# humeniuka/semiclassical

Hardware: AMD Instinct MI355X
Metric: trajectory-steps/sec + wall-time to converged C(t), anharmonic-AS D=60 (higher is better)
Workload: dtype f64

## Files before the change

### include/semiclassical_hip.h

```cpp
#ifndef SEMICLASSICAL_HIP_H
#define SEMICLASSICAL_HIP_H

#include <stdint.h>

#ifdef __cplusplus
extern "C" {
#endif

#define SC_ABI_VERSION        18

#define SC_OK                 0
#define SC_ERR_BAD_ARGUMENT  -1
#define SC_ERR_UNSUPPORTED   -2
#define SC_ERR_LAUNCH        -3

#define SC_POT_MORSE          1
#define SC_POT_HARMONIC_SEP   2
#define SC_POT_EPS_MORSE      3
#define SC_POT_HARMONIC_DENSE 4

typedef struct sc_potential {
    int32_t kind;
    int32_t dim;
    const double *par0;
// ... 71 lines not shown
    double *ksum;
    double *ssum;
} sc_dense_scratch;

int         sc_version(void);
const char *sc_last_error(void);
int sc_abi_version(void);
int sc_struct_size(const char *name);
int sc_tuning_build(void);

int sc_step_grid(int64_t n, int32_t dim);
int sc_correlate_grid(int64_t n, int32_t dim);

int sc_mono_convert(const sc_state *st, int32_t to_layout, void *stream);

int sc_state_from_reference(const double *y, const sc_state *st, void *stream);
int sc_state_to_reference(const sc_state *st, double *y, void *stream);

int sc_sample_initial(const sc_state *st, const double *ilz, const double *z0, int32_t dprime, double prob0,
                      uint64_t seed, uint64_t subsequence, int64_t first, int32_t init_state, double *zi_t,
                      double *probi, double *xi_out, void *stream);

int sc_hk_step(const sc_potential *pot, const sc_state *st, const sc_hk_consts *hk,
               double dt, int32_t mode, double *energy_partials, void *stream);

typedef struct sc_multi_scratch {
    double *work, *qp_mid, *act_mid, *c2_mid, *sgn_mid;
    int32_t *unrepaired;
} sc_multi_scratch;
int sc_hk_step_multi_supported(const sc_potential *pot, const sc_state *st, const sc_hk_consts *hk);
int sc_hk_step_multi(const sc_potential *pot, const sc_state *st, const sc_hk_consts *hk, const sc_multi_scratch *ms,
                     double dt, double *energy_partials, void *stream);

int sc_overlap(const sc_overlap_consts *oc, const double *qp, int64_t n, double *out, void *stream);

int sc_nac_initial(const sc_nac_consts *nc, const double *zi, int64_t n, double *nacq, void *stream);

int sc_hk_correlate(const sc_state *st, const sc_overlap_consts *ovl_t0, const sc_nac_consts *nc,
                    const double *vi, const double *probi, const double *nacq, double mc_norm,
                    double *cq_out, double *kq_out, double *partials, void *stream);

int sc_hk_correlate_m(const sc_state *st, const sc_overlap_consts *ovl_t0, const sc_nac_consts *nc,
                      const double *vi, const double *probi, const double *nacq, double mc_norm,
                      double *cq_out, double *kq_out, double *partials, double *moment_partials, void *stream);
int sc_term_moments_grid(int64_t n);
int sc_term_moments(const double *cq, const double *kq, int64_t n, double *moment_partials, void *stream);
int sc_reduce_moments(const double *moment_partials, int32_t n_rows, double *moments, void *stream);
int sc_reduce_slot_moments_at(const double *corr_partials, int32_t n_corr, const double *moment_partials, int32_t n_mom,
                              double *slots, double *moments, int64_t *cursor, void *stream);

int sc_reduce_slot(const double *corr_partials, int32_t n_corr, const double *energy_partials, int32_t n_energy_blocks,
                   double n_energy, double *slot, void *stream);

int sc_reduce_slot_at(const double *corr_partials, int32_t n_corr, double *slots, int64_t *cursor, void *stream);

int sc_hk_run_slots(int64_t n, int32_t dim);
int sc_hk_run_supported(const sc_potential *pot, const sc_hk_consts *hk, const sc_overlap_consts *ovl_t0);
int sc_hk_run(const sc_potential *pot, const sc_state *st, const sc_hk_consts *hk, const sc_overlap_consts *ovl_t0,
              const sc_nac_consts *nc, const double *vi, const double *probi, const double *nacq, double mc_norm,
              double dt, int32_t nsteps, double *partials, double *slots_out, double *elog, void *stream);

int64_t sc_hk_run_scratch_doubles(int64_t n, int32_t dim, int32_t nsteps, int32_t moments);
int sc_hk_run_m(const sc_potential *pot, const sc_state *st, const sc_hk_consts *hk, const sc_overlap_consts *ovl_t0,
                const sc_nac_consts *nc, const double *vi, const double *probi, const double *nacq, double mc_norm,
                double dt, int32_t nsteps, double *partials, double *slots_out, double *elog, double *moments_out, void *stream);

// ... 92 lines not shown
```

### semiclassical_amd/_lib.py

```python
import ctypes as C
import os

HERE = os.path.dirname(os.path.abspath(__file__))
LIB_PATH = os.environ.get("SC_LIB_PATH") or os.path.join(HERE, "libsemiclassical_hip.so")

c_double_p = C.c_void_p


class sc_potential(C.Structure):
    _fields_ = [("kind", C.c_int32), ("dim", C.c_int32),
                ("par0", c_double_p), ("par1", c_double_p), ("par2", c_double_p),
                ("scalar0", C.c_double), ("inv_mass", c_double_p),
                ("lin_prop", c_double_p), ("lin_dt", C.c_double)]


class sc_state(C.Structure):
    _fields_ = [("n", C.c_int64), ("dim", C.c_int32), ("mono_layout", C.c_int32),
                ("qp", c_double_p), ("act", c_double_p), ("mono", c_double_p),
                ("c2", c_double_p), ("sgn", c_double_p), ("work", c_double_p), ("flags", C.c_void_p)]


class sc_hk_consts(C.Structure):
    _fields_ = [("dim", C.c_int32), ("dprime", C.c_int32), ("diag", C.c_int32), ("real_lr", C.c_int32),
                ("st", c_double_p), ("si", c_double_p),
# ... 39 lines not shown


class sc_dense_scratch(C.Structure):
    _fields_ = [("hess", c_double_p), ("kprev", c_double_p), ("ksum", c_double_p), ("ssum", c_double_p)]


SC_POT_MORSE, SC_POT_HARMONIC_SEP, SC_POT_EPS_MORSE, SC_POT_HARMONIC_DENSE = 1, 2, 3, 4
SEPARABLE_KINDS = (SC_POT_MORSE, SC_POT_HARMONIC_SEP, SC_POT_EPS_MORSE)
SC_MONO_ROWMAJOR, SC_MONO_TILED16 = 0, 1

P = C.POINTER
ABI_VERSION = 18
STRUCTS = (sc_potential, sc_state, sc_hk_consts, sc_overlap_consts, sc_nac_consts, sc_wm_consts, sc_gdml_model,
           sc_dense_scratch, sc_multi_scratch)

SIGNATURES = {
    "sc_version": (C.c_int, []),
    "sc_abi_version": (C.c_int, []),
    "sc_struct_size": (C.c_int, [C.c_char_p]),
    "sc_tuning_build": (C.c_int, []),
    "sc_last_error": (C.c_char_p, []),
    "sc_step_grid": (C.c_int, [C.c_int64, C.c_int32]),
    "sc_correlate_grid": (C.c_int, [C.c_int64, C.c_int32]),
    "sc_mono_convert": (C.c_int, [P(sc_state), C.c_int32, C.c_void_p]),
    "sc_state_from_reference": (C.c_int, [c_double_p, P(sc_state), C.c_void_p]),
    "sc_state_to_reference": (C.c_int, [P(sc_state), c_double_p, C.c_void_p]),
    "sc_sample_initial": (C.c_int, [P(sc_state), c_double_p, c_double_p, C.c_int32, C.c_double, C.c_uint64, C.c_uint64,
                                    C.c_int64, C.c_int32, c_double_p, c_double_p, c_double_p, C.c_void_p]),
    "sc_hk_step": (C.c_int, [P(sc_potential), P(sc_state), P(sc_hk_consts), C.c_double, C.c_int32,
                             c_double_p, C.c_void_p]),
    "sc_hk_step_multi_supported": (C.c_int, [P(sc_potential), P(sc_state), P(sc_hk_consts)]),
    "sc_hk_step_multi": (C.c_int, [P(sc_potential), P(sc_state), P(sc_hk_consts), P(sc_multi_scratch), C.c_double, c_double_p,
                                   C.c_void_p]),
    "sc_overlap": (C.c_int, [P(sc_overlap_consts), c_double_p, C.c_int64, c_double_p, C.c_void_p]),
    "sc_nac_initial": (C.c_int, [P(sc_nac_consts), c_double_p, C.c_int64, c_double_p, C.c_void_p]),
    "sc_hk_correlate": (C.c_int, [P(sc_state), P(sc_overlap_consts), P(sc_nac_consts), c_double_p, c_double_p,
                                  c_double_p, C.c_double, c_double_p, c_double_p, c_double_p, C.c_void_p]),
    "sc_hk_correlate_m": (C.c_int, [P(sc_state), P(sc_overlap_consts), P(sc_nac_consts), c_double_p, c_double_p,
                                    c_double_p, C.c_double, c_double_p, c_double_p, c_double_p, c_double_p, C.c_void_p]),
    "sc_term_moments_grid": (C.c_int, [C.c_int64]),
    "sc_term_moments": (C.c_int, [c_double_p, c_double_p, C.c_int64, c_double_p, C.c_void_p]),
    "sc_reduce_moments": (C.c_int, [c_double_p, C.c_int32, c_double_p, C.c_void_p]),
    "sc_reduce_slot_moments_at": (C.c_int, [c_double_p, C.c_int32, c_double_p, C.c_int32, c_double_p, c_double_p, C.c_void_p,
                                            C.c_void_p]),
    "sc_term_blocks": (C.c_int, [c_double_p, c_double_p, C.c_int64, C.c_int32, c_double_p, C.c_void_p]),
    "sc_term_blocks_at": (C.c_int, [c_double_p, c_double_p, C.c_int64, C.c_int32, c_double_p, C.c_void_p, C.c_void_p]),
    "sc_hk_run_blocks": (C.c_int, [c_double_p, C.c_int64, C.c_int32, C.c_int32, C.c_int32, c_double_p, C.c_void_p]),
    "sc_hk_run_slots": (C.c_int, [C.c_int64, C.c_int32]),
    "sc_hk_run_scratch_doubles": (C.c_int64, [C.c_int64, C.c_int32, C.c_int32, C.c_int32]),
    "sc_hk_run_m": (C.c_int, [P(sc_potential), P(sc_state), P(sc_hk_consts), P(sc_overlap_consts), P(sc_nac_consts), c_double_p,
                              c_double_p, c_double_p, C.c_double, C.c_double, C.c_int32, c_double_p, c_double_p, c_double_p,
                              c_double_p, C.c_void_p]),
    "sc_hk_run_modal_m": (C.c_int, [P(sc_potential), P(sc_state), P(sc_hk_consts), P(sc_overlap_consts), P(sc_nac_consts),
                                    c_double_p, c_double_p, c_double_p, C.c_double, C.c_double, C.c_int32, c_double_p, c_double_p,
                                    c_double_p, c_double_p, c_double_p, C.c_void_p]),
    "sc_hk_run_supported": (C.c_int, [P(sc_potential), P(sc_hk_consts), P(sc_overlap_consts)]),
    "sc_hk_run": (C.c_int, [P(sc_potential), P(sc_state), P(sc_hk_consts), P(sc_overlap_consts), P(sc_nac_consts), c_double_p,
                            c_double_p, c_double_p, C.c_double, C.c_double, C.c_int32, c_double_p, c_double_p, c_double_p,
                            C.c_void_p]),
    "sc_mono_similarity": (C.c_int, [P(sc_state), c_double_p, c_double_p, C.c_void_p]),
    "sc_hk_run_modal_supported": (C.c_int, [P(sc_potential), P(sc_hk_consts), P(sc_overlap_consts)]),
    "sc_hk_run_modal": (C.c_int, [P(sc_potential), P(sc_state), P(sc_hk_consts), P(sc_overlap_consts), P(sc_nac_consts), c_double_p,
                                  c_double_p, c_double_p, C.c_double, C.c_double, C.c_int32, c_double_p, c_double_p, c_double_p,
                                  c_double_p, C.c_void_p]),
    "sc_hk_step_modal_supported": (C.c_int, [P(sc_potential), P(sc_state), P(sc_hk_consts)]),
    "sc_hk_step_modal": (C.c_int, [P(sc_potential), P(sc_state), P(sc_hk_consts), C.c_double, C.c_int32, c_double_p, c_double_p,
# ... 90 lines not shown
```

### semiclassical_amd/csrc/sc_common.h

```cpp
#pragma once
#include <hip/hip_runtime.h>
#include <stdint.h>
#include <stdarg.h>
#include <stdio.h>
#include <stdlib.h>

#include "semiclassical_hip.h"

#define SC_HBAR 1.0

typedef double2 cplx;

__device__ __forceinline__ cplx c_make(double re, double im) { return make_double2(re, im); }
__device__ __forceinline__ cplx c_add(cplx a, cplx b) { return make_double2(a.x + b.x, a.y + b.y); }
__device__ __forceinline__ cplx c_sub(cplx a, cplx b) { return make_double2(a.x - b.x, a.y - b.y); }
__device__ __forceinline__ cplx c_mul(cplx a, cplx b) {
    return make_double2(a.x * b.x - a.y * b.y, a.x * b.y + a.y * b.x);
}
__device__ __forceinline__ cplx c_scale(cplx a, double s) { return make_double2(a.x * s, a.y * s); }
__device__ __forceinline__ cplx c_conj(cplx a) { return make_double2(a.x, -a.y); }
__device__ __forceinline__ double c_abs2(cplx a) { return a.x * a.x + a.y * a.y; }
__device__ __forceinline__ cplx c_inv(cplx a) {
    double s = 1.0 / c_abs2(a);
    return make_double2(a.x * s, -a.y * s);
// ... 160 lines not shown
    q = q + h6 * (kq1 + 2.0 * kq2 + 2.0 * kq3 + kq4);
    p = p + h6 * (kp1 + 2.0 * kp2 + 2.0 * kp3 + kp4);
}

__device__ __forceinline__ void sep_row_propagator(double im, double h1, double h2, double h3, double h4, double dt,
                                                   double &p11, double &p12, double &p21, double &p22) {
    p11 = 1.0; p21 = 0.0; p12 = 0.0; p22 = 1.0;
    rk4_pair(p11, p21, im, h1, h2, h3, h4, dt);
    rk4_pair(p12, p22, im, h1, h2, h3, h4, dt);
}

__device__ __forceinline__ void sep_propagate_row(double p11, double p12, double p21, double p22,
                                                  double &mqq, double &mqp, double &mpq, double &mpp) {
    const double nqq = fma(p12, mpq, p11 * mqq), npq = fma(p22, mpq, p21 * mqq);
    const double nqp = fma(p12, mpp, p11 * mqp), npp = fma(p22, mpp, p21 * mqp);
    mqq = nqq; mpq = npq; mqp = nqp; mpp = npp;
}

__device__ __forceinline__ cplx prefactor_element_diag(double sta, double ista, double sib, double isib,
                                                       double mqq, double mqp, double mpq, double mpp) {
    return c_make(0.5 * (sta * isib * mqq + ista * sib * mpp),
                  0.5 * (-SC_HBAR * sta * sib * mqp + (1.0 / SC_HBAR) * ista * isib * mpq));
}

__device__ __forceinline__ bool crossed_branch_cut(cplx prev, cplx det) {
    return prev.x < 0.0 && det.x < 0.0 && prev.y * det.y < 0.0;
}

__host__ __device__ __forceinline__ int sc_error_block(int64_t i, int B) { return (int)((i >> 2) & (B - 1)); }
__host__ __device__ __forceinline__ bool sc_error_blocks_valid(int B) { return B >= 2 && B <= 64 && (B & (B - 1)) == 0; }

#define SC_SEP16_MAX_D 12
int sc_launch_step_sep16(const StepArgs &a, int grid_entries, hipStream_t s);
int sc_launch_step_sd_multi(const StepArgs &a, const sc_multi_scratch &ms, hipStream_t s);
int sc_launch_step_lin(const StepArgs &a, int grid, hipStream_t s);

int sc_fail(int code, const char *fmt, ...);
int sc_check_launch(const char *what);
int sc_require_rowmajor(const sc_state *st, const char *who);
```

### semiclassical_amd/csrc/sc_hk_step.hip

```cpp
#include "sc_common.h"
#include "sc_prefactor.h"

namespace {

__device__ __forceinline__ size_t align2(size_t x) { return (x + 1) & ~size_t(1); }

template <bool DENSE>
__global__ __launch_bounds__(256) void hk_step_kernel(StepArgs A) {
    extern __shared__ double2 smem2[];
    double *smem = (double *)smem2;
    const int D = A.st.dim, DD = D * D, tid = threadIdx.x, nth = blockDim.x;
    const int dp = A.hk.dprime;
    const bool diag = A.hk.diag != 0;
    const bool fixup = (A.mode & 0x200) != 0;
    if (fixup && A.st.flags[A.st.n] == 0) return;
    const bool do_step = (A.mode & 0xff) == 0 && !fixup;
    const bool init_track = (A.mode & 0xff) == 1;
    const double dt = A.dt, hh = 0.5 * dt, h6 = dt / 6.0;

    size_t off = 0;
    double *red = smem + off;  off += 32;
    int *ipiv = (int *)(smem + off); off += 2;
    double *hst = smem + off;  off += align2(4 * D);
    double *vec = smem + off;  off += align2(4 * D);
// ... 235 lines not shown
            return sc_check_launch("sc_hk_step (flag counter)");
        const int rc = sc_launch_step_lin(a, grid, s);
        if (rc < 0) return rc;
        if (rc != 0) {
            if (!st->flags) return SC_OK;
            a.mode = mode | 0x200;
            a.epart = nullptr;
            if (hipFuncSetAttribute((const void *)hk_step_kernel<true>, hipFuncAttributeMaxDynamicSharedMemorySize, (int)lds) != hipSuccess)
                return sc_check_launch("sc_hk_step (LDS attribute)");
            hipLaunchKernelGGL(hk_step_kernel<true>, dim3(grid), dim3(threads), lds, s, a);
            return sc_check_launch("sc_hk_step (fix-up)");
        }
    }
    if (dense) {
        if (hipFuncSetAttribute((const void *)hk_step_kernel<true>, hipFuncAttributeMaxDynamicSharedMemorySize,
                                (int)lds) != hipSuccess)
            return sc_check_launch("sc_hk_step (LDS attribute)");
        hipLaunchKernelGGL(hk_step_kernel<true>, dim3(grid), dim3(threads), lds, s, a);
    } else {
        if (hipFuncSetAttribute((const void *)hk_step_kernel<false>, hipFuncAttributeMaxDynamicSharedMemorySize,
                                (int)lds) != hipSuccess)
            return sc_check_launch("sc_hk_step (LDS attribute)");
        hipLaunchKernelGGL(hk_step_kernel<false>, dim3(grid), dim3(threads), lds, s, a);
    }
    return sc_check_launch("sc_hk_step");
}

extern "C" int sc_hk_step_multi_supported(const sc_potential *pot, const sc_state *st, const sc_hk_consts *hk) {
    if (!pot || !st || !hk) return 0;
    return sc_pot_is_separable(pot->kind) && hk->diag && hk->dprime == st->dim && pot->dim == st->dim && hk->dim == st->dim && st->dim > 16 && st->dim <= 64 &&
           st->mono_layout == SC_MONO_TILED16 && st->work && st->flags ? 1 : 0;
}

extern "C" int sc_hk_step_multi(const sc_potential *pot, const sc_state *st, const sc_hk_consts *hk, const sc_multi_scratch *ms,
                                double dt, double *energy_partials, void *stream) {
    if (!pot || !st || !hk || !ms) return sc_fail(SC_ERR_BAD_ARGUMENT, "sc_hk_step_multi: null argument");
    if (!ms->work || !ms->qp_mid || !ms->act_mid || !ms->c2_mid || !ms->sgn_mid || !ms->unrepaired)
        return sc_fail(SC_ERR_BAD_ARGUMENT, "sc_hk_step_multi: null scratch field");
    if (!sc_hk_step_multi_supported(pot, st, hk))
        return sc_fail(SC_ERR_UNSUPPORTED, "sc_hk_step_multi: needs a separable potential, diagonal width matrices, 16 < D <= 64, the tiled "
                       "storage order (sc_mono_convert) and sc_state.work / flags (use sc_hk_step)");
    if (st->n <= 0) return SC_OK;
    hipStream_t s = (hipStream_t)stream;
    if (hipMemsetAsync(st->flags + st->n, 0, 2 * sizeof(int32_t), s) != hipSuccess) return sc_check_launch("sc_hk_step_multi (flag counter)");
    const int grid = sc_step_grid(st->n, st->dim);
    StepArgs a{*pot, *st, *hk, dt, 0, energy_partials, 2 * grid};
    int rc = sc_launch_step_sd_multi(a, *ms, s);
    if (rc != SC_OK) return rc;
    return sc_hk_step(pot, st, hk, dt, 0x400, nullptr, stream);
}
```

### semiclassical_amd/csrc/sc_hk_step_sd.hip

```cpp
#include <algorithm>
#include "sc_common.h"
#include "sc_hk_lu.h"
#include "sc_row16.h"

#ifndef SC_SD_DEPTH
#define SC_SD_DEPTH 1
#endif
#ifndef SC_SD_XPREFETCH
#define SC_SD_XPREFETCH 1
#endif
#ifndef SC_SD_XPREFETCH2
#define SC_SD_XPREFETCH2 1
#endif
#ifndef SC_SD_XPREFETCH_AHEAD
#define SC_SD_XPREFETCH_AHEAD 1
#endif
#ifndef SC_SD_LOAD_AUX
#define SC_SD_LOAD_AUX 2
#endif
#ifndef SC_SD_MULTI_LOAD_AUX
#define SC_SD_MULTI_LOAD_AUX 2
#endif
#ifndef SC_SD_NOSTORE_LOAD_AUX
#define SC_SD_NOSTORE_LOAD_AUX 0
// ... 20 lines not shown
#define SC_SD_BLOCK_BARRIER no_barrier
#endif

namespace {

typedef unsigned int sc_v2u __attribute__((ext_vector_type(2)));
typedef unsigned int sc_v4u __attribute__((ext_vector_type(4)));

struct MultiArgs {
    const double *work;
    double *c2_mid, *sgn_mid;
    int *unrepaired;
};

#ifdef SD_PHASE_CLOCK
__device__ unsigned long long *g_sd_clock = nullptr;
#define SD_TICK(i)                                                                                                       \
    do {                                                                                                                 \
        if (pc_blk >= 0 && pc_item < 256 && (threadIdx.x & 63) == 0)                                                     \
            g_sd_clock[((pc_blk * 4 + (threadIdx.x >> 6)) * 256 + pc_item) * 6 + (i)] = wall_clock64();                  \
    } while (0)
#else
#define SD_TICK(i) do { } while (0)
#endif

template <int NR, int MINW, bool STEP, bool TILED, int KS = 1>
__global__ __launch_bounds__(256, MINW) void hk_step_sd_kernel(StepArgs A, MultiArgs MA) {
#ifdef SD_PHASE_CLOCK
    const int pc_blk = g_sd_clock == nullptr ? -1 : (blockIdx.x == 0 ? 0 : (blockIdx.x == 512 ? 1 : -1));
    int pc_item = 0;
#endif
    constexpr bool mid_store = KS > 1 && NR < SC_SD_NOSTORE_MIN_NR;
    constexpr int NP = mid_store ? 1 : KS;
    constexpr int aux_first = KS == 1 ? SC_SD_LOAD_AUX : (mid_store ? SC_SD_MULTI_LOAD_AUX : SC_SD_NOSTORE_LOAD_AUX);
    __shared__ double prop[NP][4 * 64];
    __shared__ double scl[4 * 64];
    __shared__ cplx rowbuf[16][64];
    __shared__ PivotRecord pivrec[16];
    __shared__ cplx detbuf[2][16 * NR];
    __shared__ int weakbuf[2];
    __shared__ int nextbuf[2];

    static_assert(KS == 1 || !SC_SD_DIRECT_P || NR < SC_SD_NOSTORE_MIN_NR, "a later sub-step of a visit needs the row propagators of the earlier ones (prop[])");
    const int D = A.st.dim, DD = D * D, tid = threadIdx.x;
    constexpr bool do_step = STEP;
    constexpr int NCL_BASE = 16 * (NR - 1);
    if (tid < 64) {
        const bool in = tid < D;
        const double st = in ? A.hk.st[tid] : 1.0, si = in ? A.hk.si[tid] : 1.0;
        if (tid < 16) pivrec[tid].pad = 0;
        if (tid < 2) { nextbuf[tid] = 0; weakbuf[tid] = 0; }
        scl[tid] = st; scl[64 + tid] = 1.0 / st; scl[128 + tid] = si; scl[192 + tid] = 1.0 / si;
#pragma unroll
        for (int k = 0; k < NP; ++k) { prop[k][tid] = 1.0; prop[k][64 + tid] = 0.0; prop[k][128 + tid] = 0.0; prop[k][192 + tid] = 1.0; }
    }
    __syncthreads();

    const bool rows_odd = row_order_is_odd(D);
    const int wave_s = __builtin_amdgcn_readfirstlane(tid >> 6);
    int seq0 = 0;
    int par = 0;
    double raw[2][4][NR];
    double pv[2][4] = {{1.0, 0.0, 0.0, 1.0}, {1.0, 0.0, 0.0, 1.0}};
    double prv = 0.0;
    bool first = true;
    int *cursor = A.st.flags ? A.st.flags + A.st.n + 1 : nullptr;
// ... 110 lines not shown
                if (do_step) {
                    sep_propagate_row(p11, p12, p21, p22, mqq, mqp, mpq, mpp);
                    const double out[4] = {mqq, mqp, mpq, mpp};
                    if constexpr (!store_blocks) {
                        (void)out; (void)rs; (void)vofs; (void)base; (void)plane;
                        __builtin_amdgcn_sched_barrier(0);
                    } else if constexpr (TILED) {
#pragma unroll
                        for (int pp = 0; pp < 2; ++pp) {
                            sc_v4u v;
                            v.x = (unsigned)__double2loint(out[2 * pp]); v.y = (unsigned)__double2hiint(out[2 * pp]);
                            v.z = (unsigned)__double2loint(out[2 * pp + 1]); v.w = (unsigned)__double2hiint(out[2 * pp + 1]);
                            __builtin_amdgcn_raw_buffer_store_b128(v, rs, vofs, base + pp * 2 * plane, aux_store);
                            __builtin_amdgcn_sched_barrier(0);
                            __asm__ volatile("s_nop 2");
                            __builtin_amdgcn_sched_barrier(0);
                        }
                    } else {
#pragma unroll
                        for (int pl = 0; pl < 4; ++pl) {
                            sc_v2u v;
                            v.x = (unsigned)__double2loint(out[pl]); v.y = (unsigned)__double2hiint(out[pl]);
                            __builtin_amdgcn_raw_buffer_store_b64(v, rs, vofs, base + pl * plane, 0);
                        }
                    }
                }
                const int bl = (16 * rb + tjl) & 63;
                const double sib = scl[128 + bl], isib = scl[192 + bl];
                m[ra][rb] = prefactor_element_diag(sta, ista, sib, isib, mqq, mqp, mpq, mpp);
                __asm__ volatile("" : "+v"(m[ra][rb].x), "+v"(m[ra][rb].y));
            }
        };
        SD_TICK(0);
        if (first || !SC_SD_XPREFETCH || NR == 1) first_requests(tr, ksc);
        first = false;
        __builtin_amdgcn_sched_barrier(0);
        if (NR > 1 && SC_SD_DEPTH > 1) load_slot(std::integral_constant<int, (NR > 1 ? 1 : 0)>(), tr, std::integral_constant<int, aux_load>());
        __builtin_amdgcn_sched_barrier(0);
        if (do_step && !SC_SD_DIRECT_P) {
            if (pa < D) prop[mid_store ? 0 : ks][64 * pk + pa] = prv;
            __syncthreads();
        }
        sfor<0, NR>([&](auto rac) {
            constexpr int ra = decltype(rac)::value;
            if (SC_SD_DEPTH == 1 && ra > (SC_SD_XPREFETCH2 ? 1 : 0)) load_slot(rac, tr, std::integral_constant<int, aux_load>());
            if (SC_SD_DEPTH > 1 && ra + 1 < NR && ra > 0) load_slot(std::integral_constant<int, (ra + 1 < NR ? ra + 1 : 0)>(), tr, std::integral_constant<int, aux_load>());
            __builtin_amdgcn_sched_barrier(0);
            finish_slot(rac);
            __builtin_amdgcn_sched_barrier(0);
        });

        constexpr bool skip_lu = SC_SD_ABLATE_LU != 0;
        SD_TICK(1);
        if (ks == 0 && cursor && tl == 0) nextbuf[par] = drawn;
        __syncthreads();
        SD_TICK(2);
        auto wg_barrier = [] { __syncthreads(); };
        auto no_barrier = [] {};
        (void)no_barrier; (void)wg_barrier;
        sfor<0, NR>([&](auto kbc) {
            constexpr int KB = decltype(kbc)::value;
            if (ks == 0 && KB == (NR > 1 ? 1 : 0)) {
                if (NR > 1) trn = cursor ? (int64_t)gridDim.x + __builtin_amdgcn_readfirstlane(nextbuf[par]) : tr + gridDim.x;
            }
            if (SC_SD_XPREFETCH && NR > 1 && KB == (NR - SC_SD_XPREFETCH_AHEAD > 1 ? NR - SC_SD_XPREFETCH_AHEAD : 1)) {
                const int64_t tnext = ks + 1 < KS ? tr : trn;
                if (tnext < A.st.n) {
                    first_requests(tnext, std::integral_constant<int, ksn>());
                } else {
                    prv = 0.0;
#pragma unroll
                    for (int pl = 0; pl < 4; ++pl) {
                        pv[0][pl] = 0.0;
#pragma unroll
                        for (int rb = 0; rb < NR; ++rb) {
                            raw[0][pl][rb] = 0.0;
                            if (SC_SD_XPREFETCH2) raw[1][pl][rb] = 0.0;
                        }
                    }
                }
            }
            if (!skip_lu) {
                if (KB == 0) eliminate_block<NR, KB, 64>(m, detbuf[par], D, seq0 + 1 + KB, rowbuf, pivrec, weak, tl, no_barrier);
                else eliminate_block<NR, KB, 64>(m, detbuf[par], D, seq0 + 1 + KB, rowbuf, pivrec, weak, tl, SC_SD_BLOCK_BARRIER);
            }
        });
        SD_TICK(3);
        __syncthreads();
        SD_TICK(4);
        if (ks == 0 && NR == 1) trn = cursor ? (int64_t)gridDim.x + __builtin_amdgcn_readfirstlane(nextbuf[par]) : tr + gridDim.x;
        cplx *c2 = (cplx *)A.st.c2;
        const cplx *c2_in = ks == 0 ? c2 + tr : (const cplx *)MA.c2_mid + ((int64_t)(ks - 1) * A.st.n + tr);
        const double *sg_in = ks == 0 ? A.st.sgn + tr : MA.sgn_mid + ((int64_t)(ks - 1) * A.st.n + tr);
        cplx *c2_out = ks == KS - 1 ? c2 + tr : (cplx *)MA.c2_mid + ((int64_t)ks * A.st.n + tr);
        double *sg_out = ks == KS - 1 ? A.st.sgn + tr : MA.sgn_mid + ((int64_t)ks * A.st.n + tr);
        if (tl < 16) lu_partial_products<NR>(detbuf[par], tl);
        if (ks == KS - 1 && tl == 0 && (*weak & 1) && A.st.flags && !skip_lu) {
            if (KS > 1) {
                c2[tr] = *c2_in;
                A.st.sgn[tr] = *sg_in;
            }
// ... 256 lines not shown
    const bool step = (a.mode & 0xff) == 0;
    const bool tiled = a.st.mono_layout == SC_MONO_TILED16;
#ifdef SC_TUNING
    if (nr == 4 && step && a.mode == 0 && getenv("SC_WS")) return sc_launch_step_ws(a, s);
#endif
    int sdgrid = grid;
#ifdef SC_TUNING
    if (const char *g = getenv("SC_SD_GRID")) sdgrid = (int)std::min<int64_t>(a.st.n, atoi(g));
#endif
#define SC_LAUNCH_SD(NR_, OCC_)                                                                                         \
    do {                                                                                                                \
        if (step && tiled) hipLaunchKernelGGL((hk_step_sd_kernel<NR_, OCC_, true, true>), dim3(sdgrid), dim3(256), 0, s, a, MultiArgs{});   \
        else if (step) hipLaunchKernelGGL((hk_step_sd_kernel<NR_, OCC_, true, false>), dim3(sdgrid), dim3(256), 0, s, a, MultiArgs{});     \
        else if (tiled) hipLaunchKernelGGL((hk_step_sd_kernel<NR_, OCC_, false, true>), dim3(sdgrid), dim3(256), 0, s, a, MultiArgs{});    \
        else hipLaunchKernelGGL((hk_step_sd_kernel<NR_, OCC_, false, false>), dim3(sdgrid), dim3(256), 0, s, a, MultiArgs{});              \
    } while (0)
    switch (nr) {
        case 1: SC_LAUNCH_SD(1, 4); break;
        case 2: SC_LAUNCH_SD(2, 4); break;
        case 3: SC_LAUNCH_SD(3, 4); break;
        default:
#ifdef SC_TUNING
            if (occ == 3) { SC_LAUNCH_SD(4, 3); break; }
            if (occ < 3) { SC_LAUNCH_SD(4, 2); break; }
#endif
            (void)occ;
            SC_LAUNCH_SD(4, 4);
            break;
    }
#undef SC_LAUNCH_SD
    return sc_check_launch("sc_hk_step (separable/diagonal fast path)");
}

int sc_launch_step_sd_multi(const StepArgs &a, const sc_multi_scratch &ms, hipStream_t s) {
    const int D = a.st.dim, nr = (D + 15) / 16, grid = sc_step_grid(a.st.n, D);
    ModesMultiArgs mm{ms.work, ms.qp_mid, ms.act_mid};
    hipLaunchKernelGGL(hk_modes_multi_kernel<2>, dim3(grid), dim3(256), 0, s, a, mm);
    int rc = sc_check_launch("sc_hk_step_multi (modes)");
    if (rc) return rc;
    MultiArgs ma{ms.work, ms.c2_mid, ms.sgn_mid, ms.unrepaired};
    switch (nr) {
        case 2: hipLaunchKernelGGL((hk_step_sd_kernel<2, 4, true, true, 2>), dim3(grid), dim3(256), 0, s, a, ma); break;
        case 3: hipLaunchKernelGGL((hk_step_sd_kernel<3, 4, true, true, 2>), dim3(grid), dim3(256), 0, s, a, ma); break;
        case 4:
#ifdef SC_TUNING
            if (const char *occ_env = getenv("SC_SD_OCC")) {
                if (atoi(occ_env) == 3) { hipLaunchKernelGGL((hk_step_sd_kernel<4, 3, true, true, 2>), dim3(grid), dim3(256), 0, s, a, ma); break; }
                if (atoi(occ_env) == 2) { hipLaunchKernelGGL((hk_step_sd_kernel<4, 2, true, true, 2>), dim3(grid), dim3(256), 0, s, a, ma); break; }
            }
#endif
            hipLaunchKernelGGL((hk_step_sd_kernel<4, 4, true, true, 2>), dim3(grid), dim3(256), 0, s, a, ma); break;
        default: return sc_fail(SC_ERR_UNSUPPORTED, "sc_hk_step_multi: D = %d", D);
    }
    return sc_check_launch("sc_hk_step_multi (two steps per visit)");
}

#ifdef LU_PIVOT_CLOCK
extern "C" int sc_lu_pivot_clock(unsigned long long *buf) {
    return hipMemcpyToSymbol(HIP_SYMBOL(g_lu_clock), &buf, sizeof(buf)) == hipSuccess ? 0 : -3;
}
#endif
```

### semiclassical_amd/propagators.py

```python
import logging

import numpy as np
import torch

from . import _lib, hostmath
from ._lib import (lib, check, ptr, sc_state, sc_hk_consts, sc_overlap_consts, sc_nac_consts, sc_wm_consts,
                   sc_dense_scratch, sc_multi_scratch)
from .units import hbar

__all__ = ['HermanKlukPropagator', 'WaltonManolopoulosPropagator']

logger = logging.getLogger(__name__)

C128 = torch.complex128
F64 = torch.float64


def _potential_fingerprint(potential):
    d = potential.dimensions()
    probe = torch.zeros((d, 1), dtype=F64)
    other = (0.05 + 0.1 * torch.arange(1, d + 1, dtype=F64) / d).reshape(d, 1)
    masses = hostmath.as_f64(potential.masses())
    tau1 = hostmath.as_f64(potential.derivative_coupling_1st(probe))[:, 0]
    tau2 = hostmath.as_f64(potential.derivative_coupling_2nd(probe))[:, 0]
# ... 497 lines not shown

    def run(self, potential, dt, nt, energy0_es=0.0, slots=None, use_graph=False, moments=None, standard_errors=False, blocks=None):
        assert self.dim == potential.dimensions(), "potential has wrong dimensions"
        dt = float(dt)
        self._remember_nac(potential)
        own = slots is None
        if standard_errors and not own:
            raise ValueError("standard_errors=True returns the errors of run()'s own slots: pass moments= together with slots")
        if own:
            slots = torch.zeros((nt, 5), dtype=F64, device=self.device)
            if standard_errors and moments is None:
                moments = torch.zeros((nt, 6), dtype=F64, device=self.device)
        else:
            self._check_slots(slots, nt)
        if moments is not None:
            self._check_slots(moments, nt, width=6, name="moments")
        nblocks = None if blocks is None else self._check_blocks(blocks, nt)
        bbase = None if blocks is None else blocks.data_ptr()
        brow = (lambda k: None) if bbase is None else (lambda k: (bbase + 32 * nblocks * k, nblocks))
        t0 = self.t
        base = slots.data_ptr()
        mbase = None if moments is None else moments.data_ptr()
        mrow = (lambda k: None) if mbase is None else (lambda k: mbase + 48 * k)
        fused = (hasattr(potential, "_descriptor") and not hasattr(potential, "_gdml_model") and self.dim <= 64
                 and self._nac_generic is None)
        desc = self._potential_descriptor(potential, dt) if fused else None
        if fused and self._whole_loop_applies(desc):
            self._run_whole_loop(desc, dt, nt, slots, potential, moments, blocks)
        elif (use_graph and fused and nt > 2 and not getattr(self, "profile_step_kernel", False) and not self.kernel_timing
              and self._modal_step_constants(potential, desc, dt) is None):
            self._run_graph(potential, dt, nt, desc, slots, mbase, brow(0))
        else:
            pairs = fused and nt >= 2 and self._multi_applies(desc)
            k = 0
            while k < nt:
                self._launch_correlate(base + 40 * k, per_trajectory=False, slot_row=slots[k], mom_ptr=mrow(k), blk=brow(k))
                if pairs and k + 1 < nt:
                    self._launch_step_pair(desc, dt)
                    self._launch_correlate(base + 40 * (k + 1), per_trajectory=False, state=self._multi["state_mid"],
                                           mom_ptr=mrow(k + 1), blk=brow(k + 1))
                    self.t += dt
                    self.t += dt
                    k += 2
                else:
                    self._launch_step(potential, dt, desc=desc, remembered=True)
                    self.t += dt
                    k += 1
        self._corr_step = -1
        if not own:
            return None
        self.synchronize()
        if standard_errors:
            return self.finalize_slots(slots, t0, dt, energy0_es) + self.finalize_moments(slots, moments, t0, dt, energy0_es,
                                                                                          self._ntraj_norm)
        return self.finalize_slots(slots, t0, dt, energy0_es)

    def standard_errors(self, energy0_es=0.0):
        slot = torch.zeros((1, 5), dtype=F64, device=self.device)
        mom = torch.zeros((1, 6), dtype=F64, device=self.device)
        self._launch_correlate(slot.data_ptr(), slot_row=slot[0], mom_ptr=mom.data_ptr())
        self.synchronize()
        sc, sk = self.finalize_moments(slot, mom, self.t, 0.0, energy0_es, self._ntraj_norm)
        return complex(sc[0]), complex(sk[0])

    _whole_loop_ok = True

    def _whole_loop_applies(self, desc):
        return (self._whole_loop_ok and not self.kernel_timing and not getattr(self, "profile_step_kernel", False)
                and not self._shortcut_applies(desc)
                and bool(lib.sc_hk_run_supported(desc, self._hk, self._ovl_t0)))

    normal_modes_from = 16

    def _modal_constants(self, potential, desc, dt):
        if (desc.kind != _lib.SC_POT_HARMONIC_DENSE or self._pre.diag or not hasattr(potential, "_normal_modes")
                or not self._hk.real_lr or not lib.sc_hk_run_modal_supported(desc, self._hk, self._ovl_t0)):
# ... 78 lines not shown
        self._set_mono_layout(_lib.SC_MONO_ROWMAJOR)
        chunk = min(nt, 512)
        mom = moments is not None
        partials = torch.empty(lib.sc_hk_run_scratch_doubles(self.ntraj, self.dim, chunk, int(mom)), dtype=F64, device=self.device)
        nac = self._nac
        modal = self._modal_constants(potential, desc, dt) if nt >= self.normal_modes_from else None
        if modal is not None:
            self._to_normal_modes(modal, forward=True)
        for k0 in range(0, nt, chunk):
            k = min(chunk, nt - k0)
            tail = (ptr(partials), slots.data_ptr() + 40 * k0, ptr(self._elog), self._stream())
            head = (self._ovl_t0, nac, ptr(self._vi), ptr(self.probi), ptr(self._nacq) if nac is not None else None, self._mc_norm(), dt, k)
            if mom:
                tail = tail[:3] + (C_void(moments.data_ptr() + 48 * k0), tail[3])
            if modal is not None:
                run = lib.sc_hk_run_modal_m if mom else lib.sc_hk_run_modal
                check(run(desc, self._state, modal["hk"], *head, ptr(modal["phi"]), *tail))
            else:
                run = lib.sc_hk_run_m if mom else lib.sc_hk_run
                check(run(desc, self._state, self._hk, *head, *tail))
            if blocks is not None:
                nblocks = blocks.shape[1]
                check(lib.sc_hk_run_blocks(ptr(partials), self.ntraj, self.dim, k, nblocks,
                                           C_void(blocks.data_ptr() + 32 * nblocks * k0), self._stream()))
        if modal is not None:
            self._to_normal_modes(modal, forward=False)
        self._run_scratch = partials
        self._nsteps += nt
        for _ in range(nt):
            self.t += dt

    _multi_ok = True
    pair_steps = True

    def _multi_applies(self, desc):
        if not (self._multi_ok and self.pair_steps and self._blocks_structurally_diagonal and self._nac_generic is None
                and not self._shortcut_applies(desc) and self._fast_path_layout(desc) == _lib.SC_MONO_TILED16):
            return False
        probe = sc_state.from_buffer_copy(self._state)
        probe.mono_layout = _lib.SC_MONO_TILED16
        return bool(lib.sc_hk_step_multi_supported(desc, probe, self._hk))

    def _launch_step_pair(self, desc, dt):
        n, d, dev = self.ntraj, self.dim, self.device
        if self._multi is None:
            grid = self._gstep
            bufs = {"work": torch.empty((2, n, 4, d), dtype=F64, device=dev), "qp": torch.empty((n, 2 * d), dtype=F64, device=dev),
                    "act": torch.empty(n, dtype=F64, device=dev), "c2": torch.empty(n, dtype=C128, device=dev),
                    "sgn": torch.empty(n, dtype=F64, device=dev), "bad": torch.zeros(1, dtype=torch.int32, device=dev),
                    "epart": torch.zeros((2, grid), dtype=F64, device=dev)}
            bufs["ms"] = sc_multi_scratch(work=ptr(bufs["work"]), qp_mid=ptr(bufs["qp"]), act_mid=ptr(bufs["act"]), c2_mid=ptr(bufs["c2"]),
                                          sgn_mid=ptr(bufs["sgn"]), unrepaired=ptr(bufs["bad"]))
            mid = sc_state.from_buffer_copy(self._state)
            mid.qp, mid.act, mid.c2, mid.sgn = ptr(bufs["qp"]), ptr(bufs["act"]), ptr(bufs["c2"]), ptr(bufs["sgn"])
            bufs["state_mid"] = mid
            self._multi = bufs
        m = self._multi
        s = self._stream()
        self._leave_modal()
        self._sync_dense_mono(leave_diagonal=True)
        self._set_mono_layout(_lib.SC_MONO_TILED16)
        m["state_mid"].mono_layout = _lib.SC_MONO_TILED16
        timed = getattr(self, "profile_step_kernel", False)
        if timed:
            e0, e1 = torch.cuda.Event(enable_timing=True), torch.cuda.Event(enable_timing=True)
            e0.record()
        with self._timed("hk_step_pair"):
            check(lib.sc_hk_step_multi(desc, self._state, self._hk, m["ms"], dt, ptr(m["epart"]), s))
        if timed:
            e1.record()
            self.__dict__.setdefault("_step_events", []).append((e0, e1, 2))
        for sub in range(2):
            check(lib.sc_energy_guard(C_void(m["epart"].data_ptr() + 8 * sub * self._gstep), self._gstep, float(n), ptr(self._elog), s))
        self._nsteps += 2

    def _run_graph(self, potential, dt, nt, desc, slots, mbase=None, blk=None):
        base = slots.data_ptr()
        cursor = torch.zeros(1, dtype=torch.int64, device=self.device)

        def iteration():
            self._launch_correlate(base, per_trajectory=False, cursor=cursor, mom_ptr=mbase, blk=blk)
            self._launch_step(potential, dt, desc=desc, remembered=True)
        iteration()
        graph = torch.cuda.CUDAGraph()
        steps_before = self._nsteps
        with torch.cuda.graph(graph):
            iteration()
        self._nsteps = steps_before + 1
        graph.replay()
        for _ in range(nt - 2):
            graph.replay()
            self._nsteps += 1
        for _ in range(nt):
            self.t += dt
        if hasattr(self, "_wm_step"):
            self._wm_step = self._nsteps
        self._graph = graph

    def _check_slots(self, slots, nt, width=5, name="slots"):
        if not (isinstance(slots, torch.Tensor) and slots.dtype == F64 and slots.dim() == 2 and slots.shape[1] == width
                and slots.shape[0] >= nt and slots.is_contiguous() and slots.device == self.device):
            raise ValueError(f"{name} has to be a contiguous float64 tensor of shape (>= {nt}, {width}) on {self.device}, got "
                             f"{getattr(slots, 'dtype', type(slots))} {tuple(getattr(slots, 'shape', ()))} on "
                             f"{getattr(slots, 'device', '?')}")

    def _check_blocks(self, blocks, nt):
        if not (isinstance(blocks, torch.Tensor) and blocks.dtype == F64 and blocks.dim() == 3 and blocks.shape[2] == 4
# ... 419 lines not shown
```

Measured before the change: 28.88 million.

## Advance three or four HK steps per kernel visit for large D

Generalises the paired-step fused kernel to 3 or 4 steps per visit (KS template) for 32 < D <= 64. This amortises monodromy-matrix loads and stores across more steps per launch. It adds a late prefetch of the propagator work slice for KS >= 4. Python drives the new path by default (visit_steps=3) when the state is large enough, and allocates extra mid-step scratch states for the intermediate correlate calls. The cost is more scratch memory and register pressure in the larger kernel instantiations.

```diff
diff --git a/include/semiclassical_hip.h b/include/semiclassical_hip.h
--- a/include/semiclassical_hip.h
+++ b/include/semiclassical_hip.h
@@ -127,6 +127,10 @@
 int sc_hk_step_multi(const sc_potential *pot, const sc_state *st, const sc_hk_consts *hk, const sc_multi_scratch *ms,
                      double dt, double *energy_partials, void *stream);
 
+int sc_hk_step_visit_supported(const sc_potential *pot, const sc_state *st, const sc_hk_consts *hk, int32_t ksteps);
+int sc_hk_step_visit(const sc_potential *pot, const sc_state *st, const sc_hk_consts *hk, const sc_multi_scratch *ms,
+                     double dt, double *energy_partials, int32_t ksteps, void *stream);
+
 int sc_overlap(const sc_overlap_consts *oc, const double *qp, int64_t n, double *out, void *stream);
 
 int sc_nac_initial(const sc_nac_consts *nc, const double *zi, int64_t n, double *nacq, void *stream);
diff --git a/semiclassical_amd/_lib.py b/semiclassical_amd/_lib.py
--- a/semiclassical_amd/_lib.py
+++ b/semiclassical_amd/_lib.py
@@ -95,6 +95,9 @@
     "sc_hk_step_multi_supported": (C.c_int, [P(sc_potential), P(sc_state), P(sc_hk_consts)]),
     "sc_hk_step_multi": (C.c_int, [P(sc_potential), P(sc_state), P(sc_hk_consts), P(sc_multi_scratch), C.c_double, c_double_p,
                                    C.c_void_p]),
+    "sc_hk_step_visit_supported": (C.c_int, [P(sc_potential), P(sc_state), P(sc_hk_consts), C.c_int32]),
+    "sc_hk_step_visit": (C.c_int, [P(sc_potential), P(sc_state), P(sc_hk_consts), P(sc_multi_scratch), C.c_double, c_double_p,
+                                   C.c_int32, C.c_void_p]),
     "sc_overlap": (C.c_int, [P(sc_overlap_consts), c_double_p, C.c_int64, c_double_p, C.c_void_p]),
     "sc_nac_initial": (C.c_int, [P(sc_nac_consts), c_double_p, C.c_int64, c_double_p, C.c_void_p]),
     "sc_hk_correlate": (C.c_int, [P(sc_state), P(sc_overlap_consts), P(sc_nac_consts), c_double_p, c_double_p,
diff --git a/semiclassical_amd/csrc/sc_common.h b/semiclassical_amd/csrc/sc_common.h
--- a/semiclassical_amd/csrc/sc_common.h
+++ b/semiclassical_amd/csrc/sc_common.h
@@ -216,7 +216,7 @@
 
 #define SC_SEP16_MAX_D 12
 int sc_launch_step_sep16(const StepArgs &a, int grid_entries, hipStream_t s);
-int sc_launch_step_sd_multi(const StepArgs &a, const sc_multi_scratch &ms, hipStream_t s);
+int sc_launch_step_sd_multi(const StepArgs &a, const sc_multi_scratch &ms, int ksteps, hipStream_t s);
 int sc_launch_step_lin(const StepArgs &a, int grid, hipStream_t s);
 
 int sc_fail(int code, const char *fmt, ...);
diff --git a/semiclassical_amd/csrc/sc_hk_step.hip b/semiclassical_amd/csrc/sc_hk_step.hip
--- a/semiclassical_amd/csrc/sc_hk_step.hip
+++ b/semiclassical_amd/csrc/sc_hk_step.hip
@@ -291,20 +291,35 @@
            st->mono_layout == SC_MONO_TILED16 && st->work && st->flags ? 1 : 0;
 }
 
-extern "C" int sc_hk_step_multi(const sc_potential *pot, const sc_state *st, const sc_hk_consts *hk, const sc_multi_scratch *ms,
-                                double dt, double *energy_partials, void *stream) {
-    if (!pot || !st || !hk || !ms) return sc_fail(SC_ERR_BAD_ARGUMENT, "sc_hk_step_multi: null argument");
+static int hk_step_visit(const char *who, const sc_potential *pot, const sc_state *st, const sc_hk_consts *hk, const sc_multi_scratch *ms,
+                         double dt, double *energy_partials, int ksteps, void *stream) {
+    if (!pot || !st || !hk || !ms) return sc_fail(SC_ERR_BAD_ARGUMENT, "%s: null argument", who);
     if (!ms->work || !ms->qp_mid || !ms->act_mid || !ms->c2_mid || !ms->sgn_mid || !ms->unrepaired)
-        return sc_fail(SC_ERR_BAD_ARGUMENT, "sc_hk_step_multi: null scratch field");
-    if (!sc_hk_step_multi_supported(pot, st, hk))
-        return sc_fail(SC_ERR_UNSUPPORTED, "sc_hk_step_multi: needs a separable potential, diagonal width matrices, 16 < D <= 64, the tiled "
-                       "storage order (sc_mono_convert) and sc_state.work / flags (use sc_hk_step)");
+        return sc_fail(SC_ERR_BAD_ARGUMENT, "%s: null scratch field", who);
+    if (!sc_hk_step_visit_supported(pot, st, hk, ksteps))
+        return sc_fail(SC_ERR_UNSUPPORTED, "%s: needs a separable potential, diagonal width matrices, 16 < D <= 64 (more than two steps per "
+                       "visit: 32 < D, at most four), the tiled storage order (sc_mono_convert) and sc_state.work / flags (use sc_hk_step)", who);
     if (st->n <= 0) return SC_OK;
     hipStream_t s = (hipStream_t)stream;
     if (hipMemsetAsync(st->flags + st->n, 0, 2 * sizeof(int32_t), s) != hipSuccess) return sc_check_launch("sc_hk_step_multi (flag counter)");
     const int grid = sc_step_grid(st->n, st->dim);
-    StepArgs a{*pot, *st, *hk, dt, 0, energy_partials, 2 * grid};
-    int rc = sc_launch_step_sd_multi(a, *ms, s);
+    StepArgs a{*pot, *st, *hk, dt, 0, energy_partials, ksteps * grid};
+    int rc = sc_launch_step_sd_multi(a, *ms, ksteps, s);
     if (rc != SC_OK) return rc;
     return sc_hk_step(pot, st, hk, dt, 0x400, nullptr, stream);
 }
+
+extern "C" int sc_hk_step_multi(const sc_potential *pot, const sc_state *st, const sc_hk_consts *hk, const sc_multi_scratch *ms,
+                                double dt, double *energy_partials, void *stream) {
+    return hk_step_visit("sc_hk_step_multi", pot, st, hk, ms, dt, energy_partials, 2, stream);
+}
+
+extern "C" int sc_hk_step_visit_supported(const sc_potential *pot, const sc_state *st, const sc_hk_consts *hk, int32_t ksteps) {
+    if (ksteps < 2 || ksteps > 4 || !sc_hk_step_multi_supported(pot, st, hk)) return 0;
+    return ksteps == 2 || st->dim > 32 ? 1 : 0;
+}
+
+extern "C" int sc_hk_step_visit(const sc_potential *pot, const sc_state *st, const sc_hk_consts *hk, const sc_multi_scratch *ms,
+                                double dt, double *energy_partials, int32_t ksteps, void *stream) {
+    return hk_step_visit("sc_hk_step_visit", pot, st, hk, ms, dt, energy_partials, ksteps, stream);
+}
diff --git a/semiclassical_amd/csrc/sc_hk_step_sd.hip b/semiclassical_amd/csrc/sc_hk_step_sd.hip
--- a/semiclassical_amd/csrc/sc_hk_step_sd.hip
+++ b/semiclassical_amd/csrc/sc_hk_step_sd.hip
@@ -76,6 +76,7 @@
 #endif
     constexpr bool mid_store = KS > 1 && NR < SC_SD_NOSTORE_MIN_NR;
     constexpr int NP = mid_store ? 1 : KS;
+    constexpr bool late_p = KS >= 4 && NR >= 4;
     constexpr int aux_first = KS == 1 ? SC_SD_LOAD_AUX : (mid_store ? SC_SD_MULTI_LOAD_AUX : SC_SD_NOSTORE_LOAD_AUX);
     __shared__ double prop[NP][4 * 64];
     __shared__ double scl[4 * 64];
@@ -252,6 +253,9 @@
             }
         };
         SD_TICK(0);
+        if constexpr (late_p) {
+            if (!first && do_step && pa < Dl) prv = MA.work[(((int64_t)ks * A.st.n + tr) * 4 + pk) * (int64_t)Dl + pa];
+        }
         if (first || !SC_SD_XPREFETCH || NR == 1) first_requests(tr, ksc);
         first = false;
         __builtin_amdgcn_sched_barrier(0);
@@ -286,7 +290,13 @@
             if (SC_SD_XPREFETCH && NR > 1 && KB == (NR - SC_SD_XPREFETCH_AHEAD > 1 ? NR - SC_SD_XPREFETCH_AHEAD : 1)) {
                 const int64_t tnext = ks + 1 < KS ? tr : trn;
                 if (tnext < A.st.n) {
-                    first_requests(tnext, std::integral_constant<int, ksn>());
+                    if constexpr (late_p) {
+                        constexpr int auxn = ksn == 0 ? aux_first : SC_SD_MULTI_MID_AUX;
+                        load_slot(std::integral_constant<int, 0>(), tnext, std::integral_constant<int, auxn>());
+                        if (SC_SD_XPREFETCH2) load_slot(std::integral_constant<int, 1>(), tnext, std::integral_constant<int, auxn>());
+                    } else {
+                        first_requests(tnext, std::integral_constant<int, ksn>());
+                    }
                 } else {
                     prv = 0.0;
 #pragma unroll
@@ -609,7 +619,26 @@
     return sc_check_launch("sc_hk_step (separable/diagonal fast path)");
 }
 
-int sc_launch_step_sd_multi(const StepArgs &a, const sc_multi_scratch &ms, hipStream_t s) {
+template <int KS>
+static int launch_step_sd_visit(const StepArgs &a, const sc_multi_scratch &ms, hipStream_t s) {
+    const int D = a.st.dim, nr = (D + 15) / 16, grid = sc_step_grid(a.st.n, D);
+    ModesMultiArgs mm{ms.work, ms.qp_mid, ms.act_mid};
+    hipLaunchKernelGGL(hk_modes_multi_kernel<KS>, dim3(grid), dim3(256), 0, s, a, mm);
+    int rc = sc_check_launch("sc_hk_step_visit (modes)");
+    if (rc) return rc;
+    MultiArgs ma{ms.work, ms.c2_mid, ms.sgn_mid, ms.unrepaired};
+    switch (nr) {
+        case 3: hipLaunchKernelGGL((hk_step_sd_kernel<3, 4, true, true, KS>), dim3(grid), dim3(256), 0, s, a, ma); break;
+        case 4: hipLaunchKernelGGL((hk_step_sd_kernel<4, 4, true, true, KS>), dim3(grid), dim3(256), 0, s, a, ma); break;
+        default: return sc_fail(SC_ERR_UNSUPPORTED, "sc_hk_step_visit: %d steps per visit at D = %d", KS, D);
+    }
+    return sc_check_launch("sc_hk_step_visit (KS steps per visit)");
+}
+
+int sc_launch_step_sd_multi(const StepArgs &a, const sc_multi_scratch &ms, int ksteps, hipStream_t s) {
+    if (ksteps == 3) return launch_step_sd_visit<3>(a, ms, s);
+    if (ksteps == 4) return launch_step_sd_visit<4>(a, ms, s);
+    if (ksteps != 2) return sc_fail(SC_ERR_UNSUPPORTED, "sc_hk_step_visit: %d steps per visit", ksteps);
     const int D = a.st.dim, nr = (D + 15) / 16, grid = sc_step_grid(a.st.n, D);
     ModesMultiArgs mm{ms.work, ms.qp_mid, ms.act_mid};
     hipLaunchKernelGGL(hk_modes_multi_kernel<2>, dim3(grid), dim3(256), 0, s, a, mm);
diff --git a/semiclassical_amd/propagators.py b/semiclassical_amd/propagators.py
--- a/semiclassical_amd/propagators.py
+++ b/semiclassical_amd/propagators.py
@@ -553,16 +553,26 @@
             self._run_graph(potential, dt, nt, desc, slots, mbase, brow(0))
         else:
             pairs = fused and nt >= 2 and self._multi_applies(desc)
+            kmax = self._visit_steps_for(desc) if pairs else 1
             k = 0
             while k < nt:
                 self._launch_correlate(base + 40 * k, per_trajectory=False, slot_row=slots[k], mom_ptr=mrow(k), blk=brow(k))
-                if pairs and k + 1 < nt:
+                ks = min(kmax, nt - k) if pairs else 1
+                if ks == 2:
                     self._launch_step_pair(desc, dt)
                     self._launch_correlate(base + 40 * (k + 1), per_trajectory=False, state=self._multi["state_mid"],
                                            mom_ptr=mrow(k + 1), blk=brow(k + 1))
                     self.t += dt
                     self.t += dt
                     k += 2
+                elif ks > 2:
+                    self._launch_step_visit(desc, dt, ks)
+                    for j in range(1, ks):
+                        self._launch_correlate(base + 40 * (k + j), per_trajectory=False, state=self._multi["states_mid"][j - 1],
+                                               mom_ptr=mrow(k + j), blk=brow(k + j))
+                    for _ in range(ks):
+                        self.t += dt
+                    k += ks
                 else:
                     self._launch_step(potential, dt, desc=desc, remembered=True)
                     self.t += dt
@@ -707,6 +717,8 @@
 
     _multi_ok = True
     pair_steps = True
+    visit_steps = 3
+    visit_min_bytes = 256 << 20
 
     def _multi_applies(self, desc):
         if not (self._multi_ok and self.pair_steps and self._blocks_structurally_diagonal and self._nac_generic is None
@@ -716,38 +728,68 @@
         probe.mono_layout = _lib.SC_MONO_TILED16
         return bool(lib.sc_hk_step_multi_supported(desc, probe, self._hk))
 
+    def _visit_steps_for(self, desc):
+        ks = int(self.visit_steps) if 32 * self.dim * self.dim * self.ntraj >= self.visit_min_bytes else 2
+        probe = sc_state.from_buffer_copy(self._state)
+        probe.mono_layout = _lib.SC_MONO_TILED16
+        while ks > 2 and not lib.sc_hk_step_visit_supported(desc, probe, self._hk, ks):
+            ks -= 1
+        return max(ks, 2)
+
+    def _visit_scratch(self, ks):
+        n, d, dev = self.ntraj, self.dim, self.device
+        m = self._multi
+        if m is not None and m["ks"] >= ks:
+            return m
+        grid = self._gstep
+        bufs = {"ks": ks, "work": torch.empty((ks, n, 4, d), dtype=F64, device=dev),
+                "qp": torch.empty(((ks - 1) * n, 2 * d), dtype=F64, device=dev),
+                "act": torch.empty((ks - 1) * n, dtype=F64, device=dev), "c2": torch.empty((ks - 1) * n, dtype=C128, device=dev),
+                "sgn": torch.empty((ks - 1) * n, dtype=F64, device=dev),
+                "bad": m["bad"] if m is not None else torch.zeros(1, dtype=torch.int32, device=dev),
+                "epart": torch.zeros((ks, grid), dtype=F64, device=dev)}
+        bufs["ms"] = sc_multi_scratch(work=ptr(bufs["work"]), qp_mid=ptr(bufs["qp"]), act_mid=ptr(bufs["act"]), c2_mid=ptr(bufs["c2"]),
+                                      sgn_mid=ptr(bufs["sgn"]), unrepaired=ptr(bufs["bad"]))
+        mids = []
+        for j in range(ks - 1):
+            mid = sc_state.from_buffer_copy(self._state)
+            mid.qp, mid.act = ptr(bufs["qp"][j * n:]), ptr(bufs["act"][j * n:])
+            mid.c2, mid.sgn = ptr(bufs["c2"][j * n:]), ptr(bufs["sgn"][j * n:])
+            mids.append(mid)
+        bufs["states_mid"], bufs["state_mid"] = mids, mids[0]
+        if m is not None:
+            bufs["retired"] = m
+        self._multi = bufs
+        return bufs
+
     def _launch_step_pair(self, desc, dt):
-        n, d, dev = self.ntraj, self.dim, self.device
-        if self._multi is None:
-            grid = self._gstep
-            bufs = {"work": torch.empty((2, n, 4, d), dtype=F64, device=dev), "qp": torch.empty((n, 2 * d), dtype=F64, device=dev),
-                    "act": torch.empty(n, dtype=F64, device=dev), "c2": torch.empty(n, dtype=C128, device=dev),
-                    "sgn": torch.empty(n, dtype=F64, device=dev), "bad": torch.zeros(1, dtype=torch.int32, device=dev),
-                    "epart": torch.zeros((2, grid), dtype=F64, device=dev)}
-            bufs["ms"] = sc_multi_scratch(work=ptr(bufs["work"]), qp_mid=ptr(bufs["qp"]), act_mid=ptr(bufs["act"]), c2_mid=ptr(bufs["c2"]),
-                                          sgn_mid=ptr(bufs["sgn"]), unrepaired=ptr(bufs["bad"]))
-            mid = sc_state.from_buffer_copy(self._state)
-            mid.qp, mid.act, mid.c2, mid.sgn = ptr(bufs["qp"]), ptr(bufs["act"]), ptr(bufs["c2"]), ptr(bufs["sgn"])
-            bufs["state_mid"] = mid
-            self._multi = bufs
-        m = self._multi
+        self._launch_step_visit(desc, dt, 2)
+
+    def _launch_step_visit(self, desc, dt, ks):
+        n = self.ntraj
+        m = self._visit_scratch(ks)
         s = self._stream()
         self._leave_modal()
         self._sync_dense_mono(leave_diagonal=True)
         self._set_mono_layout(_lib.SC_MONO_TILED16)
-        m["state_mid"].mono_layout = _lib.SC_MONO_TILED16
+        for mid in m["states_mid"]:
+            mid.mono_layout = _lib.SC_MONO_TILED16
         timed = getattr(self, "profile_step_kernel", False)
         if timed:
             e0, e1 = torch.cuda.Event(enable_timing=True), torch.cuda.Event(enable_timing=True)
             e0.record()
-        with self._timed("hk_step_pair"):
-            check(lib.sc_hk_step_multi(desc, self._state, self._hk, m["ms"], dt, ptr(m["epart"]), s))
+        if ks == 2:
+            with self._timed("hk_step_pair"):
+                check(lib.sc_hk_step_multi(desc, self._state, self._hk, m["ms"], dt, ptr(m["epart"]), s))
+        else:
+            with self._timed("hk_step_visit"):
+                check(lib.sc_hk_step_visit(desc, self._state, self._hk, m["ms"], dt, ptr(m["epart"]), ks, s))
         if timed:
             e1.record()
-            self.__dict__.setdefault("_step_events", []).append((e0, e1, 2))
-        for sub in range(2):
+            self.__dict__.setdefault("_step_events", []).append((e0, e1, ks))
+        for sub in range(ks):
             check(lib.sc_energy_guard(C_void(m["epart"].data_ptr() + 8 * sub * self._gstep), self._gstep, float(n), ptr(self._elog), s))
-        self._nsteps += 2
+        self._nsteps += ks
 
     def _run_graph(self, potential, dt, nt, desc, slots, mbase=None, blk=None):
         base = slots.data_ptr()
```

Measured after the change: 29.38 million, median of 6. 1.7% higher.
